# dusk-network/schnorr

Measured on NVIDIA B200. Metric: verifies_per_s, higher is better.
Workload: dtype u32

## Files before the change

### schnorr_b200/csrc/fq.cuh

```cuda
#pragma once
#include <cstdint>

#include "constants_gen.cuh"

#if defined(__CUDACC__)
#define SB_HD __host__ __device__ __forceinline__
#define SB_D __device__ __forceinline__
#else
#define SB_HD inline
#define SB_D inline
#endif

namespace sb200 {

#ifndef SB_Q1_SHORTCUT
#define SB_Q1_SHORTCUT 0
#endif

struct fq {
  uint32_t v[8];
};

#if !defined(__CUDA_ARCH__)
namespace emu {
// ... 60 lines not shown
      : "r"(a), "r"(b0), "r"(b2), "r"(b4), "r"(b6));
#else
  SB_COUNT(wide, 4);
  uint32_t c = emu::add_at(x, 8, 0, (uint64_t)a * b0, 0);
  c += emu::add_at(x, 8, 2, (uint64_t)a * b2, 0);
  c += emu::add_at(x, 8, 4, (uint64_t)a * b4, 0);
  c += emu::add_at(x, 8, 6, (uint64_t)a * b6, 0);
  ytop += c;
#endif
}

SB_HD void blk_mac_odd(uint32_t* y, uint32_t a, uint32_t b1, uint32_t b3, uint32_t b5, uint32_t b7) {
#if defined(__CUDA_ARCH__)
  asm("mad.lo.cc.u32 %0, %8, %9, %0;\n\t"
      "madc.hi.cc.u32 %1, %8, %9, %1;\n\t"
      "madc.lo.cc.u32 %2, %8, %10, %2;\n\t"
      "madc.hi.cc.u32 %3, %8, %10, %3;\n\t"
      "madc.lo.cc.u32 %4, %8, %11, %4;\n\t"
      "madc.hi.cc.u32 %5, %8, %11, %5;\n\t"
      "madc.lo.cc.u32 %6, %8, %12, %6;\n\t"
      "madc.hi.u32 %7, %8, %12, %7;"
      : "+r"(y[0]), "+r"(y[1]), "+r"(y[2]), "+r"(y[3]), "+r"(y[4]), "+r"(y[5]), "+r"(y[6]), "+r"(y[7])
      : "r"(a), "r"(b1), "r"(b3), "r"(b5), "r"(b7));
#else
  SB_COUNT(wide, 4);
  uint32_t c = emu::add_at(y, 8, 0, (uint64_t)a * b1, 0);
  c += emu::add_at(y, 8, 2, (uint64_t)a * b3, 0);
  c += emu::add_at(y, 8, 4, (uint64_t)a * b5, 0);
  c += emu::add_at(y, 8, 6, (uint64_t)a * b7, 0);
  (void)c;
#endif
}

SB_HD void blk_red_even_q(uint32_t* x, uint32_t& ytop, uint32_t m, uint32_t q2, uint32_t q4, uint32_t q6) {
#if defined(__CUDA_ARCH__)
  asm("mad.lo.cc.u32 %0, %7, %8, %0;\n\t"
      "madc.hi.cc.u32 %1, %7, %8, %1;\n\t"
      "madc.lo.cc.u32 %2, %7, %9, %2;\n\t"
      "madc.hi.cc.u32 %3, %7, %9, %3;\n\t"
      "madc.lo.cc.u32 %4, %7, %10, %4;\n\t"
      "madc.hi.cc.u32 %5, %7, %10, %5;\n\t"
      "addc.u32 %6, %6, 0;"
      : "+r"(x[2]), "+r"(x[3]), "+r"(x[4]), "+r"(x[5]), "+r"(x[6]), "+r"(x[7]), "+r"(ytop)
      : "r"(m), "r"(q2), "r"(q4), "r"(q6));
#else
  SB_COUNT(wide, 3);
  uint32_t c = emu::add_at(x, 8, 2, (uint64_t)m * q2, 0);
  c += emu::add_at(x, 8, 4, (uint64_t)m * q4, 0);
  c += emu::add_at(x, 8, 6, (uint64_t)m * q6, 0);
  ytop += c;
#endif
}

SB_HD void blk_red_odd_q(uint32_t* y, uint32_t m, uint32_t t0, uint32_t q3, uint32_t q5, uint32_t q7) {
#if defined(__CUDA_ARCH__)
  asm("{\n\t.reg .u32 h;\n\t"
      "min.u32 h, %8, 1;\n\t"
      "sub.u32 h, %8, h;\n\t"
      "add.cc.u32 %0, %0, %9;\n\t"
      "addc.cc.u32 %1, %1, h;\n\t"
      "madc.lo.cc.u32 %2, %8, %10, %2;\n\t"
      "madc.hi.cc.u32 %3, %8, %10, %3;\n\t"
      "madc.lo.cc.u32 %4, %8, %11, %4;\n\t"
      "madc.hi.cc.u32 %5, %8, %11, %5;\n\t"
      "madc.lo.cc.u32 %6, %8, %12, %6;\n\t"
      "madc.hi.u32 %7, %8, %12, %7;\n\t}"
      : "+r"(y[0]), "+r"(y[1]), "+r"(y[2]), "+r"(y[3]), "+r"(y[4]), "+r"(y[5]), "+r"(y[6]), "+r"(y[7])
      : "r"(m), "r"(t0), "r"(q3), "r"(q5), "r"(q7));
#else
  SB_COUNT(wide, 3);
  uint32_t hi1 = m - (m != 0 ? 1u : 0u);
  uint32_t c = emu::add_at(y, 8, 0, ((uint64_t)hi1 << 32) | t0, 0);
  c += emu::add_at(y, 8, 2, (uint64_t)m * q3, 0);
  c += emu::add_at(y, 8, 4, (uint64_t)m * q5, 0);
  c += emu::add_at(y, 8, 6, (uint64_t)m * q7, 0);
  (void)c;
#endif
}

SB_HD void blk_mac1c(uint32_t* acc, uint32_t a, uint32_t b0) {
#if defined(__CUDA_ARCH__)
  asm("mad.lo.cc.u32 %0, %3, %4, %0;\n\t"
      "madc.hi.cc.u32 %1, %3, %4, %1;\n\t"
      "addc.u32 %2, %2, 0;"
      : "+r"(acc[0]), "+r"(acc[1]), "+r"(acc[2])
      : "r"(a), "r"(b0));
#else
  SB_COUNT(wide, 1);
  acc[2] += emu::add_at(acc, 2, 0, (uint64_t)a * b0, 0);
#endif
}
SB_HD void blk_mac2c(uint32_t* acc, uint32_t a, uint32_t b0, uint32_t b1) {
#if defined(__CUDA_ARCH__)
  asm("mad.lo.cc.u32 %0, %5, %6, %0;\n\t"
      "madc.hi.cc.u32 %1, %5, %6, %1;\n\t"
      "madc.lo.cc.u32 %2, %5, %7, %2;\n\t"
      "madc.hi.cc.u32 %3, %5, %7, %3;\n\t"
      "addc.u32 %4, %4, 0;"
      : "+r"(acc[0]), "+r"(acc[1]), "+r"(acc[2]), "+r"(acc[3]), "+r"(acc[4])
      : "r"(a), "r"(b0), "r"(b1));
#else
  SB_COUNT(wide, 2);
  uint32_t c = emu::add_at(acc, 4, 0, (uint64_t)a * b0, 0);
  c += emu::add_at(acc, 4, 2, (uint64_t)a * b1, 0);
  acc[4] += c;
#endif
}
SB_HD void blk_mac3c(uint32_t* acc, uint32_t a, uint32_t b0, uint32_t b1, uint32_t b2) {
#if defined(__CUDA_ARCH__)
  asm("mad.lo.cc.u32 %0, %7, %8, %0;\n\t"
      "madc.hi.cc.u32 %1, %7, %8, %1;\n\t"
      "madc.lo.cc.u32 %2, %7, %9, %2;\n\t"
      "madc.hi.cc.u32 %3, %7, %9, %3;\n\t"
      "madc.lo.cc.u32 %4, %7, %10, %4;\n\t"
      "madc.hi.cc.u32 %5, %7, %10, %5;\n\t"
      "addc.u32 %6, %6, 0;"
      : "+r"(acc[0]), "+r"(acc[1]), "+r"(acc[2]), "+r"(acc[3]), "+r"(acc[4]), "+r"(acc[5]), "+r"(acc[6])
      : "r"(a), "r"(b0), "r"(b1), "r"(b2));
#else
  SB_COUNT(wide, 3);
  uint32_t c = emu::add_at(acc, 6, 0, (uint64_t)a * b0, 0);
  c += emu::add_at(acc, 6, 2, (uint64_t)a * b1, 0);
  c += emu::add_at(acc, 6, 4, (uint64_t)a * b2, 0);
  acc[6] += c;
#endif
}
SB_HD void blk_mac4c(uint32_t* acc, uint32_t a, uint32_t b0, uint32_t b1, uint32_t b2, uint32_t b3) {
  blk_mac_even(acc, acc[8], a, b0, b1, b2, b3);
}

SB_HD void blk_sqr_diag(uint32_t* t, const uint32_t* a) {
#if defined(__CUDA_ARCH__)
  asm("mad.lo.cc.u32 %0, %16, %16, %0;\n\t"
      "madc.hi.cc.u32 %1, %16, %16, %1;\n\t"
      "madc.lo.cc.u32 %2, %17, %17, %2;\n\t"
      "madc.hi.cc.u32 %3, %17, %17, %3;\n\t"
      "madc.lo.cc.u32 %4, %18, %18, %4;\n\t"
      "madc.hi.cc.u32 %5, %18, %18, %5;\n\t"
      "madc.lo.cc.u32 %6, %19, %19, %6;\n\t"
      "madc.hi.cc.u32 %7, %19, %19, %7;\n\t"
      "madc.lo.cc.u32 %8, %20, %20, %8;\n\t"
      "madc.hi.cc.u32 %9, %20, %20, %9;\n\t"
      "madc.lo.cc.u32 %10, %21, %21, %10;\n\t"
      "madc.hi.cc.u32 %11, %21, %21, %11;\n\t"
      "madc.lo.cc.u32 %12, %22, %22, %12;\n\t"
      "madc.hi.cc.u32 %13, %22, %22, %13;\n\t"
      "madc.lo.cc.u32 %14, %23, %23, %14;\n\t"
      "madc.hi.u32 %15, %23, %23, %15;"
      : "+r"(t[0]), "+r"(t[1]), "+r"(t[2]), "+r"(t[3]), "+r"(t[4]), "+r"(t[5]), "+r"(t[6]), "+r"(t[7]), "+r"(t[8]),
        "+r"(t[9]), "+r"(t[10]), "+r"(t[11]), "+r"(t[12]), "+r"(t[13]), "+r"(t[14]), "+r"(t[15])
      : "r"(a[0]), "r"(a[1]), "r"(a[2]), "r"(a[3]), "r"(a[4]), "r"(a[5]), "r"(a[6]), "r"(a[7]));
#else
  SB_COUNT(wide, 8);
  uint32_t c = 0;
  for (int i = 0; i < 8; i++) c += emu::add_at(t, 16, 2 * i, (uint64_t)a[i] * a[i], 0);
  (void)c;
#endif
}

SB_HD void merge_eo16(uint32_t* r, const uint32_t* e, const uint32_t* o) {
#if defined(__CUDA_ARCH__)
  r[0] = e[0];
  asm("add.cc.u32 %0, %15, %30;\n\t"
      "addc.cc.u32 %1, %16, %31;\n\t"
      "addc.cc.u32 %2, %17, %32;\n\t"
      "addc.cc.u32 %3, %18, %33;\n\t"
      "addc.cc.u32 %4, %19, %34;\n\t"
      "addc.cc.u32 %5, %20, %35;\n\t"
      "addc.cc.u32 %6, %21, %36;\n\t"
      "addc.cc.u32 %7, %22, %37;\n\t"
      "addc.cc.u32 %8, %23, %38;\n\t"
      "addc.cc.u32 %9, %24, %39;\n\t"
      "addc.cc.u32 %10, %25, %40;\n\t"
      "addc.cc.u32 %11, %26, %41;\n\t"
      "addc.cc.u32 %12, %27, %42;\n\t"
      "addc.cc.u32 %13, %28, %43;\n\t"
      "addc.u32 %14, %29, %44;"
      : "=r"(r[1]), "=r"(r[2]), "=r"(r[3]), "=r"(r[4]), "=r"(r[5]), "=r"(r[6]), "=r"(r[7]), "=r"(r[8]), "=r"(r[9]),
        "=r"(r[10]), "=r"(r[11]), "=r"(r[12]), "=r"(r[13]), "=r"(r[14]), "=r"(r[15])
      : "r"(e[1]), "r"(e[2]), "r"(e[3]), "r"(e[4]), "r"(e[5]), "r"(e[6]), "r"(e[7]), "r"(e[8]), "r"(e[9]), "r"(e[10]),
        "r"(e[11]), "r"(e[12]), "r"(e[13]), "r"(e[14]), "r"(e[15]), "r"(o[0]), "r"(o[1]), "r"(o[2]), "r"(o[3]), "r"(o[4]),
        "r"(o[5]), "r"(o[6]), "r"(o[7]), "r"(o[8]), "r"(o[9]), "r"(o[10]), "r"(o[11]), "r"(o[12]), "r"(o[13]), "r"(o[14]));
#else
  r[0] = e[0];
  uint64_t c = 0;
  for (int i = 1; i < 16; i++) {
    c += (uint64_t)e[i] + o[i - 1];
    r[i] = (uint32_t)c;
    c >>= 32;
  }
#endif
}

SB_HD uint32_t blk_fold_red_odd(uint32_t& x0, uint32_t xf, uint32_t tprev, uint32_t* y, uint32_t q1, uint32_t q3,
                                uint32_t q5, uint32_t q7) {
  uint32_t m;
#if defined(__CUDA_ARCH__)
  asm("{\n\t.reg .u32 t, h;\n\t"
      "add.cc.u32 t, %11, 0xffffffff;\n\t"
      "addc.cc.u32 %0, %0, %10;\n\t"
      "xor.b32 %9, %0, %12;\n\t"
      "add.u32 %9, %9, 1;\n\t"
      "min.u32 h, %9, 1;\n\t"
      "sub.u32 h, %9, h;\n\t"
      "addc.cc.u32 %1, %1, %0;\n\t"
      "addc.cc.u32 %2, %2, h;\n\t"
      "madc.lo.cc.u32 %3, %9, %13, %3;\n\t"
      "madc.hi.cc.u32 %4, %9, %13, %4;\n\t"
      "madc.lo.cc.u32 %5, %9, %14, %5;\n\t"
      "madc.hi.cc.u32 %6, %9, %14, %6;\n\t"
      "madc.lo.cc.u32 %7, %9, %15, %7;\n\t"
      "madc.hi.u32 %8, %9, %15, %8;\n\t}"
      : "+r"(x0), "+r"(y[0]), "+r"(y[1]), "+r"(y[2]), "+r"(y[3]), "+r"(y[4]), "+r"(y[5]), "+r"(y[6]), "+r"(y[7]), "=&r"(m)
      : "r"(xf), "r"(tprev), "r"(q1), "r"(q3), "r"(q5), "r"(q7));
#else
  SB_COUNT(wide, 4);
  uint64_t t = (uint64_t)x0 + xf + (tprev != 0 ? 1u : 0u);
  x0 = (uint32_t)t;
  uint32_t c = (uint32_t)(t >> 32);
  m = 0u - x0;
  SB_COUNT(wide, -1);
  (void)q1;
  c = emu::add_at(y, 8, 0, ((uint64_t)(m - (m != 0 ? 1u : 0u)) << 32) | x0, c);
  c += emu::add_at(y, 8, 2, (uint64_t)m * q3, 0);
  c += emu::add_at(y, 8, 4, (uint64_t)m * q5, 0);
  c += emu::add_at(y, 8, 6, (uint64_t)m * q7, 0);
  (void)c;
#endif
  return m;
}

SB_HD uint32_t add8(uint32_t* r, const uint32_t* a, const uint32_t* b) {
  uint32_t c;
#if defined(__CUDA_ARCH__)
  asm("add.cc.u32 %0, %9, %17;\n\t"
      "addc.cc.u32 %1, %10, %18;\n\t"
      "addc.cc.u32 %2, %11, %19;\n\t"
      "addc.cc.u32 %3, %12, %20;\n\t"
      "addc.cc.u32 %4, %13, %21;\n\t"
      "addc.cc.u32 %5, %14, %22;\n\t"
      "addc.cc.u32 %6, %15, %23;\n\t"
      "addc.cc.u32 %7, %16, %24;\n\t"
      "addc.u32 %8, 0, 0;"
      : "=r"(r[0]), "=r"(r[1]), "=r"(r[2]), "=r"(r[3]), "=r"(r[4]), "=r"(r[5]), "=r"(r[6]), "=r"(r[7]), "=r"(c)
      : "r"(a[0]), "r"(a[1]), "r"(a[2]), "r"(a[3]), "r"(a[4]), "r"(a[5]), "r"(a[6]), "r"(a[7]), "r"(b[0]), "r"(b[1]),
        "r"(b[2]), "r"(b[3]), "r"(b[4]), "r"(b[5]), "r"(b[6]), "r"(b[7]));
#else
  uint64_t t = 0;
  for (int i = 0; i < 8; i++) {
    t += (uint64_t)a[i] + b[i];
    r[i] = (uint32_t)t;
    t >>= 32;
  }
  c = (uint32_t)t;
#endif
  return c;
}

SB_HD void add8c(uint32_t* r, const uint32_t* a, const uint32_t* b, uint32_t t) {
#if defined(__CUDA_ARCH__)
  asm("{\n\t.reg .u32 t;\n\t"
      "add.cc.u32 t, %24, 0xffffffff;\n\t"
      "addc.cc.u32 %0, %8, %16;\n\t"
      "addc.cc.u32 %1, %9, %17;\n\t"
      "addc.cc.u32 %2, %10, %18;\n\t"
      "addc.cc.u32 %3, %11, %19;\n\t"
      "addc.cc.u32 %4, %12, %20;\n\t"
      "addc.cc.u32 %5, %13, %21;\n\t"
      "addc.cc.u32 %6, %14, %22;\n\t"
      "addc.u32 %7, %15, %23;\n\t}"
      : "=r"(r[0]), "=r"(r[1]), "=r"(r[2]), "=r"(r[3]), "=r"(r[4]), "=r"(r[5]), "=r"(r[6]), "=r"(r[7])
      : "r"(a[0]), "r"(a[1]), "r"(a[2]), "r"(a[3]), "r"(a[4]), "r"(a[5]), "r"(a[6]), "r"(a[7]), "r"(b[0]), "r"(b[1]),
        "r"(b[2]), "r"(b[3]), "r"(b[4]), "r"(b[5]), "r"(b[6]), "r"(b[7]), "r"(t));
#else
  uint64_t c = t != 0 ? 1 : 0;
  for (int i = 0; i < 8; i++) {
    c += (uint64_t)a[i] + b[i];
    r[i] = (uint32_t)c;
    c >>= 32;
  }
// ... 164 lines not shown
  return mont_reduce16(T);
#endif
  uint32_t X[8], Y[8], xf = 0, tprev = 0;
#pragma unroll
  for (int i = 0; i < 8; i++) X[i] = Y[i] = 0;
  const uint32_t q1 = SB_FQ_MOD(1), q2 = SB_FQ_MOD(2), q3 = SB_FQ_MOD(3), q4 = SB_FQ_MOD(4), q5 = SB_FQ_MOD(5),
                 q6 = SB_FQ_MOD(6), q7 = SB_FQ_MOD(7);
#pragma unroll
  for (int i = 0; i < 8; i++) {
    uint32_t ai = a.v[i];
    blk_fold_mac_odd(X[0], xf, tprev, Y, ai, b.v[1], b.v[3], b.v[5], b.v[7]);
    blk_mac_even(X, Y[7], ai, b.v[0], b.v[2], b.v[4], b.v[6]);
    tprev = X[0];
#if defined(__CUDA_ARCH__) && SB_FQ_MOD_IMM
    uint32_t m;
    asm("xor.b32 %0, %1, %2;\n\tadd.u32 %0, %0, 1;" : "=r"(m) : "r"(tprev), "r"(q1));
#else
    uint32_t m = (tprev ^ q1) + 1u;
#endif
    blk_red_even_q(X, Y[7], m, q2, q4, q6);
#if SB_Q1_SHORTCUT
    blk_red_odd_q(Y, m, tprev, q3, q5, q7);
#else
    blk_mac_odd(Y, m, q1, q3, q5, q7);
#endif
    xf = X[1];
    uint32_t nx[8], ny[8];
#pragma unroll
    for (int k = 0; k < 8; k++) nx[k] = Y[k];
#pragma unroll
    for (int k = 0; k < 6; k++) ny[k] = X[k + 2];
    ny[6] = 0;
    ny[7] = 0;
#pragma unroll
    for (int k = 0; k < 8; k++) {
      X[k] = nx[k];
      Y[k] = ny[k];
    }
  }
  fq r;
  uint32_t s[8] = {xf, Y[0], Y[1], Y[2], Y[3], Y[4], Y[5], Y[6]};
  add8c(r.v, X, s, tprev);
  cond_sub_p<FqP>(r.v);
  return r;
}

SB_HD fq mont_reduce16(const uint32_t* t) {
  uint32_t X[8], Y[8], xf = 0, tprev = 0;
#pragma unroll
  for (int i = 0; i < 8; i++) {
    X[i] = t[i];
    Y[i] = 0;
  }
  const uint32_t q1 = SB_FQ_MOD(1), q2 = SB_FQ_MOD(2), q3 = SB_FQ_MOD(3), q4 = SB_FQ_MOD(4), q5 = SB_FQ_MOD(5),
                 q6 = SB_FQ_MOD(6), q7 = SB_FQ_MOD(7);
#pragma unroll
  for (int i = 0; i < 8; i++) {
    uint32_t m = blk_fold_red_odd(X[0], xf, tprev, Y, q1, q3, q5, q7);
    tprev = X[0];
    blk_red_even_q(X, Y[7], m, q2, q4, q6);
    xf = X[1];
    uint32_t nx[8], ny[8];
#pragma unroll
    for (int k = 0; k < 8; k++) nx[k] = Y[k];
#pragma unroll
    for (int k = 0; k < 6; k++) ny[k] = X[k + 2];
    ny[6] = 0;
    ny[7] = 0;
#pragma unroll
    for (int k = 0; k < 8; k++) {
      X[k] = nx[k];
      Y[k] = ny[k];
    }
  }
  fq v, r;
  uint32_t s[8] = {xf, Y[0], Y[1], Y[2], Y[3], Y[4], Y[5], Y[6]};
  add8c(v.v, X, s, tprev);
  add8(r.v, v.v, t + 8);
  cond_sub_p<FqP>(r.v);
  return r;
}

SB_HD fq fq_sqr_inl(const fq& x) {
  SB_COUNT(fq_sqr, 1);
  const uint32_t* a = x.v;
  uint32_t E[16], O[16];
#pragma unroll
  for (int i = 0; i < 16; i++) E[i] = O[i] = 0;
  blk_mac4c(O + 0, a[0], a[1], a[3], a[5], a[7]);
  blk_mac3c(E + 2, a[0], a[2], a[4], a[6]);
  blk_mac3c(O + 2, a[1], a[2], a[4], a[6]);
  blk_mac3c(E + 4, a[1], a[3], a[5], a[7]);
  blk_mac3c(O + 4, a[2], a[3], a[5], a[7]);
  blk_mac2c(E + 6, a[2], a[4], a[6]);
  blk_mac2c(O + 6, a[3], a[4], a[6]);
  blk_mac2c(E + 8, a[3], a[5], a[7]);
  blk_mac2c(O + 8, a[4], a[5], a[7]);
  blk_mac1c(E + 10, a[4], a[6]);
  blk_mac1c(O + 10, a[5], a[6]);
  blk_mac1c(E + 12, a[5], a[7]);
  blk_mac1c(O + 12, a[6], a[7]);
  uint32_t S[16], T[16];
  merge_eo16(S, E, O);
  T[0] = S[0] << 1;
#pragma unroll
  for (int i = 1; i < 16; i++) T[i] = (S[i] << 1) | (S[i - 1] >> 31);
  blk_sqr_diag(T, a);
  return mont_reduce16(T);
}

SB_HD void mul_wide16(uint32_t* T, const uint32_t* a, const uint32_t* b) {
  uint32_t E[18], O[18];
#pragma unroll
  for (int i = 0; i < 18; i++) E[i] = O[i] = 0;
#pragma unroll
  for (int i = 0; i < 8; i++) {
    if ((i & 1) == 0) {
      blk_mac4c(E + i, a[i], b[0], b[2], b[4], b[6]);
      blk_mac4c(O + i, a[i], b[1], b[3], b[5], b[7]);
    } else {
      blk_mac4c(O + i - 1, a[i], b[0], b[2], b[4], b[6]);
      blk_mac4c(E + i + 1, a[i], b[1], b[3], b[5], b[7]);
    }
  }
  merge_eo16(T, E, O);
}

SB_HD void acc17(uint32_t* S, const uint32_t* T) {
#if defined(__CUDA_ARCH__)
  asm("add.cc.u32 %0, %0, %17;\n\t"
      "addc.cc.u32 %1, %1, %18;\n\t"
      "addc.cc.u32 %2, %2, %19;\n\t"
      "addc.cc.u32 %3, %3, %20;\n\t"
      "addc.cc.u32 %4, %4, %21;\n\t"
      "addc.cc.u32 %5, %5, %22;\n\t"
      "addc.cc.u32 %6, %6, %23;\n\t"
      "addc.cc.u32 %7, %7, %24;\n\t"
      "addc.cc.u32 %8, %8, %25;\n\t"
      "addc.cc.u32 %9, %9, %26;\n\t"
      "addc.cc.u32 %10, %10, %27;\n\t"
      "addc.cc.u32 %11, %11, %28;\n\t"
      "addc.cc.u32 %12, %12, %29;\n\t"
      "addc.cc.u32 %13, %13, %30;\n\t"
      "addc.cc.u32 %14, %14, %31;\n\t"
      "addc.cc.u32 %15, %15, %32;\n\t"
      "addc.u32 %16, %16, 0;"
      : "+r"(S[0]), "+r"(S[1]), "+r"(S[2]), "+r"(S[3]), "+r"(S[4]), "+r"(S[5]), "+r"(S[6]), "+r"(S[7]), "+r"(S[8]),
        "+r"(S[9]), "+r"(S[10]), "+r"(S[11]), "+r"(S[12]), "+r"(S[13]), "+r"(S[14]), "+r"(S[15]), "+r"(S[16])
      : "r"(T[0]), "r"(T[1]), "r"(T[2]), "r"(T[3]), "r"(T[4]), "r"(T[5]), "r"(T[6]), "r"(T[7]), "r"(T[8]), "r"(T[9]),
        "r"(T[10]), "r"(T[11]), "r"(T[12]), "r"(T[13]), "r"(T[14]), "r"(T[15]));
#else
  uint64_t c = 0;
  for (int i = 0; i < 16; i++) {
    c += (uint64_t)S[i] + T[i];
    S[i] = (uint32_t)c;
    c >>= 32;
  }
  S[16] += (uint32_t)c;
#endif
}

SB_HD fq mont_reduce17(const uint32_t* S) {
  uint32_t X[8], Y[8], xf = 0, tprev = 0;
#pragma unroll
  for (int i = 0; i < 8; i++) {
    X[i] = S[i];
    Y[i] = 0;
  }
  const uint32_t q1 = SB_FQ_MOD(1), q2 = SB_FQ_MOD(2), q3 = SB_FQ_MOD(3), q4 = SB_FQ_MOD(4), q5 = SB_FQ_MOD(5),
                 q6 = SB_FQ_MOD(6), q7 = SB_FQ_MOD(7);
#pragma unroll
  for (int i = 0; i < 8; i++) {
    uint32_t m = blk_fold_red_odd(X[0], xf, tprev, Y, q1, q3, q5, q7);
    tprev = X[0];
    blk_red_even_q(X, Y[7], m, q2, q4, q6);
    xf = X[1];
    uint32_t nx[8], ny[8];
#pragma unroll
    for (int k = 0; k < 8; k++) nx[k] = Y[k];
#pragma unroll
    for (int k = 0; k < 6; k++) ny[k] = X[k + 2];
    ny[6] = 0;
    ny[7] = 0;
#pragma unroll
    for (int k = 0; k < 8; k++) {
      X[k] = nx[k];
      Y[k] = ny[k];
    }
  }
  fq v, r;
  uint32_t s[8] = {xf, Y[0], Y[1], Y[2], Y[3], Y[4], Y[5], Y[6]};
  add8c(v.v, X, s, tprev);
  uint32_t top = S[16] + add8(r.v, v.v, S + 8);
  uint32_t t[8], q2x[8];
#pragma unroll
  for (int i = 0; i < 8; i++) q2x[i] = (FqP::p(i) << 1) | (i ? FqP::p(i - 1) >> 31 : 0u);
  uint32_t borrow = sub8(t, r.v, q2x);
  bool ge = (top != 0) | (borrow == 0);
#pragma unroll
  for (int i = 0; i < 8; i++) r.v[i] = ge ? t[i] : r.v[i];
  cond_sub_p<FqP>(r.v);
  return r;
}

SB_HD void merge_eo17(uint32_t* S, const uint32_t* E, const uint32_t* O) {
  S[0] = E[0];
#if defined(__CUDA_ARCH__)
  asm("add.cc.u32 %0, %16, %32;\n\t"
      "addc.cc.u32 %1, %17, %33;\n\t"
      "addc.cc.u32 %2, %18, %34;\n\t"
      "addc.cc.u32 %3, %19, %35;\n\t"
      "addc.cc.u32 %4, %20, %36;\n\t"
      "addc.cc.u32 %5, %21, %37;\n\t"
      "addc.cc.u32 %6, %22, %38;\n\t"
      "addc.cc.u32 %7, %23, %39;\n\t"
      "addc.cc.u32 %8, %24, %40;\n\t"
      "addc.cc.u32 %9, %25, %41;\n\t"
      "addc.cc.u32 %10, %26, %42;\n\t"
      "addc.cc.u32 %11, %27, %43;\n\t"
      "addc.cc.u32 %12, %28, %44;\n\t"
      "addc.cc.u32 %13, %29, %45;\n\t"
      "addc.cc.u32 %14, %30, %46;\n\t"
      "addc.u32 %15, %31, %47;"
      : "=r"(S[1]), "=r"(S[2]), "=r"(S[3]), "=r"(S[4]), "=r"(S[5]), "=r"(S[6]), "=r"(S[7]), "=r"(S[8]), "=r"(S[9]), "=r"(S[10]),
        "=r"(S[11]), "=r"(S[12]), "=r"(S[13]), "=r"(S[14]), "=r"(S[15]), "=r"(S[16])
      : "r"(E[1]), "r"(E[2]), "r"(E[3]), "r"(E[4]), "r"(E[5]), "r"(E[6]), "r"(E[7]), "r"(E[8]), "r"(E[9]), "r"(E[10]), "r"(E[11]),
// ... 223 lines not shown
```

Measured before the change: 28.79 million.

## Interleave field squaring with Montgomery reduction using pre-doubled operands

Replaces the separate 16-word product, doubling and diagonal pass in fq_sqr_inl with a row-by-row interleaved square-and-reduce (CIOS style). Pre-doubled limbs of a fold the cross-term doubling into the multiplicands, and the reduction helpers now return their top carry so it can be fed into the next row. This removes the merge and shift passes and the wide 16-limb intermediate, lowering register pressure and instruction count. In exchange the carry handling is more intricate, and the product terms are no longer triangular-only, so some of the squaring savings on multiplies are given up.

```diff
diff --git a/schnorr_b200/csrc/fq.cuh b/schnorr_b200/csrc/fq.cuh
--- a/schnorr_b200/csrc/fq.cuh
+++ b/schnorr_b200/csrc/fq.cuh
@@ -136,20 +136,22 @@
 #endif
 }
 
-SB_HD void blk_red_odd_q(uint32_t* y, uint32_t m, uint32_t t0, uint32_t q3, uint32_t q5, uint32_t q7) {
+SB_HD uint32_t blk_red_odd_q(uint32_t* y, uint32_t m, uint32_t t0, uint32_t q3, uint32_t q5, uint32_t q7) {
+  uint32_t ovf;
 #if defined(__CUDA_ARCH__)
   asm("{\n\t.reg .u32 h;\n\t"
-      "min.u32 h, %8, 1;\n\t"
-      "sub.u32 h, %8, h;\n\t"
-      "add.cc.u32 %0, %0, %9;\n\t"
+      "min.u32 h, %9, 1;\n\t"
+      "sub.u32 h, %9, h;\n\t"
+      "add.cc.u32 %0, %0, %10;\n\t"
       "addc.cc.u32 %1, %1, h;\n\t"
-      "madc.lo.cc.u32 %2, %8, %10, %2;\n\t"
-      "madc.hi.cc.u32 %3, %8, %10, %3;\n\t"
-      "madc.lo.cc.u32 %4, %8, %11, %4;\n\t"
-      "madc.hi.cc.u32 %5, %8, %11, %5;\n\t"
-      "madc.lo.cc.u32 %6, %8, %12, %6;\n\t"
-      "madc.hi.u32 %7, %8, %12, %7;\n\t}"
-      : "+r"(y[0]), "+r"(y[1]), "+r"(y[2]), "+r"(y[3]), "+r"(y[4]), "+r"(y[5]), "+r"(y[6]), "+r"(y[7])
+      "madc.lo.cc.u32 %2, %9, %11, %2;\n\t"
+      "madc.hi.cc.u32 %3, %9, %11, %3;\n\t"
+      "madc.lo.cc.u32 %4, %9, %12, %4;\n\t"
+      "madc.hi.cc.u32 %5, %9, %12, %5;\n\t"
+      "madc.lo.cc.u32 %6, %9, %13, %6;\n\t"
+      "madc.hi.cc.u32 %7, %9, %13, %7;\n\t"
+      "addc.u32 %8, 0, 0;\n\t}"
+      : "+r"(y[0]), "+r"(y[1]), "+r"(y[2]), "+r"(y[3]), "+r"(y[4]), "+r"(y[5]), "+r"(y[6]), "+r"(y[7]), "=r"(ovf)
       : "r"(m), "r"(t0), "r"(q3), "r"(q5), "r"(q7));
 #else
   SB_COUNT(wide, 3);
@@ -158,39 +160,40 @@
   c += emu::add_at(y, 8, 2, (uint64_t)m * q3, 0);
   c += emu::add_at(y, 8, 4, (uint64_t)m * q5, 0);
   c += emu::add_at(y, 8, 6, (uint64_t)m * q7, 0);
-  (void)c;
-#endif
-}
-
-SB_HD void blk_mac1c(uint32_t* acc, uint32_t a, uint32_t b0) {
+  ovf = c;
+#endif
+  return ovf;
+}
+
+SB_HD void blk_mac1c(uint32_t* acc, uint32_t& top, uint32_t a, uint32_t b0) {
 #if defined(__CUDA_ARCH__)
   asm("mad.lo.cc.u32 %0, %3, %4, %0;\n\t"
       "madc.hi.cc.u32 %1, %3, %4, %1;\n\t"
       "addc.u32 %2, %2, 0;"
-      : "+r"(acc[0]), "+r"(acc[1]), "+r"(acc[2])
+      : "+r"(acc[0]), "+r"(acc[1]), "+r"(top)
       : "r"(a), "r"(b0));
 #else
   SB_COUNT(wide, 1);
-  acc[2] += emu::add_at(acc, 2, 0, (uint64_t)a * b0, 0);
-#endif
-}
-SB_HD void blk_mac2c(uint32_t* acc, uint32_t a, uint32_t b0, uint32_t b1) {
+  top += emu::add_at(acc, 2, 0, (uint64_t)a * b0, 0);
+#endif
+}
+SB_HD void blk_mac2c(uint32_t* acc, uint32_t& top, uint32_t a, uint32_t b0, uint32_t b1) {
 #if defined(__CUDA_ARCH__)
   asm("mad.lo.cc.u32 %0, %5, %6, %0;\n\t"
       "madc.hi.cc.u32 %1, %5, %6, %1;\n\t"
       "madc.lo.cc.u32 %2, %5, %7, %2;\n\t"
       "madc.hi.cc.u32 %3, %5, %7, %3;\n\t"
       "addc.u32 %4, %4, 0;"
-      : "+r"(acc[0]), "+r"(acc[1]), "+r"(acc[2]), "+r"(acc[3]), "+r"(acc[4])
+      : "+r"(acc[0]), "+r"(acc[1]), "+r"(acc[2]), "+r"(acc[3]), "+r"(top)
       : "r"(a), "r"(b0), "r"(b1));
 #else
   SB_COUNT(wide, 2);
   uint32_t c = emu::add_at(acc, 4, 0, (uint64_t)a * b0, 0);
   c += emu::add_at(acc, 4, 2, (uint64_t)a * b1, 0);
-  acc[4] += c;
-#endif
-}
-SB_HD void blk_mac3c(uint32_t* acc, uint32_t a, uint32_t b0, uint32_t b1, uint32_t b2) {
+  top += c;
+#endif
+}
+SB_HD void blk_mac3c(uint32_t* acc, uint32_t& top, uint32_t a, uint32_t b0, uint32_t b1, uint32_t b2) {
 #if defined(__CUDA_ARCH__)
   asm("mad.lo.cc.u32 %0, %7, %8, %0;\n\t"
       "madc.hi.cc.u32 %1, %7, %8, %1;\n\t"
@@ -199,45 +202,61 @@
       "madc.lo.cc.u32 %4, %7, %10, %4;\n\t"
       "madc.hi.cc.u32 %5, %7, %10, %5;\n\t"
       "addc.u32 %6, %6, 0;"
-      : "+r"(acc[0]), "+r"(acc[1]), "+r"(acc[2]), "+r"(acc[3]), "+r"(acc[4]), "+r"(acc[5]), "+r"(acc[6])
+      : "+r"(acc[0]), "+r"(acc[1]), "+r"(acc[2]), "+r"(acc[3]), "+r"(acc[4]), "+r"(acc[5]), "+r"(top)
       : "r"(a), "r"(b0), "r"(b1), "r"(b2));
 #else
   SB_COUNT(wide, 3);
   uint32_t c = emu::add_at(acc, 6, 0, (uint64_t)a * b0, 0);
   c += emu::add_at(acc, 6, 2, (uint64_t)a * b1, 0);
   c += emu::add_at(acc, 6, 4, (uint64_t)a * b2, 0);
-  acc[6] += c;
+  top += c;
 #endif
 }
 SB_HD void blk_mac4c(uint32_t* acc, uint32_t a, uint32_t b0, uint32_t b1, uint32_t b2, uint32_t b3) {
   blk_mac_even(acc, acc[8], a, b0, b1, b2, b3);
 }
 
-SB_HD void blk_sqr_diag(uint32_t* t, const uint32_t* a) {
-#if defined(__CUDA_ARCH__)
-  asm("mad.lo.cc.u32 %0, %16, %16, %0;\n\t"
-      "madc.hi.cc.u32 %1, %16, %16, %1;\n\t"
-      "madc.lo.cc.u32 %2, %17, %17, %2;\n\t"
-      "madc.hi.cc.u32 %3, %17, %17, %3;\n\t"
-      "madc.lo.cc.u32 %4, %18, %18, %4;\n\t"
-      "madc.hi.cc.u32 %5, %18, %18, %5;\n\t"
-      "madc.lo.cc.u32 %6, %19, %19, %6;\n\t"
-      "madc.hi.cc.u32 %7, %19, %19, %7;\n\t"
-      "madc.lo.cc.u32 %8, %20, %20, %8;\n\t"
-      "madc.hi.cc.u32 %9, %20, %20, %9;\n\t"
-      "madc.lo.cc.u32 %10, %21, %21, %10;\n\t"
-      "madc.hi.cc.u32 %11, %21, %21, %11;\n\t"
-      "madc.lo.cc.u32 %12, %22, %22, %12;\n\t"
-      "madc.hi.cc.u32 %13, %22, %22, %13;\n\t"
-      "madc.lo.cc.u32 %14, %23, %23, %14;\n\t"
-      "madc.hi.u32 %15, %23, %23, %15;"
-      : "+r"(t[0]), "+r"(t[1]), "+r"(t[2]), "+r"(t[3]), "+r"(t[4]), "+r"(t[5]), "+r"(t[6]), "+r"(t[7]), "+r"(t[8]),
-        "+r"(t[9]), "+r"(t[10]), "+r"(t[11]), "+r"(t[12]), "+r"(t[13]), "+r"(t[14]), "+r"(t[15])
-      : "r"(a[0]), "r"(a[1]), "r"(a[2]), "r"(a[3]), "r"(a[4]), "r"(a[5]), "r"(a[6]), "r"(a[7]));
-#else
-  SB_COUNT(wide, 8);
-  uint32_t c = 0;
-  for (int i = 0; i < 8; i++) c += emu::add_at(t, 16, 2 * i, (uint64_t)a[i] * a[i], 0);
+SB_HD void blk_mac1(uint32_t* acc, uint32_t a, uint32_t b0) {
+#if defined(__CUDA_ARCH__)
+  asm("mad.lo.cc.u32 %0, %2, %3, %0;\n\t"
+      "madc.hi.u32 %1, %2, %3, %1;"
+      : "+r"(acc[0]), "+r"(acc[1])
+      : "r"(a), "r"(b0));
+#else
+  SB_COUNT(wide, 1);
+  (void)emu::add_at(acc, 2, 0, (uint64_t)a * b0, 0);
+#endif
+}
+SB_HD void blk_mac2(uint32_t* acc, uint32_t a, uint32_t b0, uint32_t b1) {
+#if defined(__CUDA_ARCH__)
+  asm("mad.lo.cc.u32 %0, %4, %5, %0;\n\t"
+      "madc.hi.cc.u32 %1, %4, %5, %1;\n\t"
+      "madc.lo.cc.u32 %2, %4, %6, %2;\n\t"
+      "madc.hi.u32 %3, %4, %6, %3;"
+      : "+r"(acc[0]), "+r"(acc[1]), "+r"(acc[2]), "+r"(acc[3])
+      : "r"(a), "r"(b0), "r"(b1));
+#else
+  SB_COUNT(wide, 2);
+  uint32_t c = emu::add_at(acc, 4, 0, (uint64_t)a * b0, 0);
+  c += emu::add_at(acc, 4, 2, (uint64_t)a * b1, 0);
+  (void)c;
+#endif
+}
+SB_HD void blk_mac3(uint32_t* acc, uint32_t a, uint32_t b0, uint32_t b1, uint32_t b2) {
+#if defined(__CUDA_ARCH__)
+  asm("mad.lo.cc.u32 %0, %6, %7, %0;\n\t"
+      "madc.hi.cc.u32 %1, %6, %7, %1;\n\t"
+      "madc.lo.cc.u32 %2, %6, %8, %2;\n\t"
+      "madc.hi.cc.u32 %3, %6, %8, %3;\n\t"
+      "madc.lo.cc.u32 %4, %6, %9, %4;\n\t"
+      "madc.hi.u32 %5, %6, %9, %5;"
+      : "+r"(acc[0]), "+r"(acc[1]), "+r"(acc[2]), "+r"(acc[3]), "+r"(acc[4]), "+r"(acc[5])
+      : "r"(a), "r"(b0), "r"(b1), "r"(b2));
+#else
+  SB_COUNT(wide, 3);
+  uint32_t c = emu::add_at(acc, 6, 0, (uint64_t)a * b0, 0);
+  c += emu::add_at(acc, 6, 2, (uint64_t)a * b1, 0);
+  c += emu::add_at(acc, 6, 4, (uint64_t)a * b2, 0);
   (void)c;
 #endif
 }
@@ -277,25 +296,27 @@
 }
 
 SB_HD uint32_t blk_fold_red_odd(uint32_t& x0, uint32_t xf, uint32_t tprev, uint32_t* y, uint32_t q1, uint32_t q3,
-                                uint32_t q5, uint32_t q7) {
+                                uint32_t q5, uint32_t q7, uint32_t& ovf) {
   uint32_t m;
 #if defined(__CUDA_ARCH__)
   asm("{\n\t.reg .u32 t, h;\n\t"
-      "add.cc.u32 t, %11, 0xffffffff;\n\t"
-      "addc.cc.u32 %0, %0, %10;\n\t"
-      "xor.b32 %9, %0, %12;\n\t"
+      "add.cc.u32 t, %12, 0xffffffff;\n\t"
+      "addc.cc.u32 %0, %0, %11;\n\t"
+      "xor.b32 %9, %0, %13;\n\t"
       "add.u32 %9, %9, 1;\n\t"
       "min.u32 h, %9, 1;\n\t"
       "sub.u32 h, %9, h;\n\t"
       "addc.cc.u32 %1, %1, %0;\n\t"
       "addc.cc.u32 %2, %2, h;\n\t"
-      "madc.lo.cc.u32 %3, %9, %13, %3;\n\t"
-      "madc.hi.cc.u32 %4, %9, %13, %4;\n\t"
-      "madc.lo.cc.u32 %5, %9, %14, %5;\n\t"
-      "madc.hi.cc.u32 %6, %9, %14, %6;\n\t"
-      "madc.lo.cc.u32 %7, %9, %15, %7;\n\t"
-      "madc.hi.u32 %8, %9, %15, %8;\n\t}"
-      : "+r"(x0), "+r"(y[0]), "+r"(y[1]), "+r"(y[2]), "+r"(y[3]), "+r"(y[4]), "+r"(y[5]), "+r"(y[6]), "+r"(y[7]), "=&r"(m)
+      "madc.lo.cc.u32 %3, %9, %14, %3;\n\t"
+      "madc.hi.cc.u32 %4, %9, %14, %4;\n\t"
+      "madc.lo.cc.u32 %5, %9, %15, %5;\n\t"
+      "madc.hi.cc.u32 %6, %9, %15, %6;\n\t"
+      "madc.lo.cc.u32 %7, %9, %16, %7;\n\t"
+      "madc.hi.cc.u32 %8, %9, %16, %8;\n\t"
+      "addc.u32 %10, 0, 0;\n\t}"
+      : "+r"(x0), "+r"(y[0]), "+r"(y[1]), "+r"(y[2]), "+r"(y[3]), "+r"(y[4]), "+r"(y[5]), "+r"(y[6]), "+r"(y[7]), "=&r"(m),
+        "=r"(ovf)
       : "r"(xf), "r"(tprev), "r"(q1), "r"(q3), "r"(q5), "r"(q7));
 #else
   SB_COUNT(wide, 4);
@@ -309,7 +330,7 @@
   c += emu::add_at(y, 8, 2, (uint64_t)m * q3, 0);
   c += emu::add_at(y, 8, 4, (uint64_t)m * q5, 0);
   c += emu::add_at(y, 8, 6, (uint64_t)m * q7, 0);
-  (void)c;
+  ovf = c;
 #endif
   return m;
 }
@@ -584,7 +605,8 @@
                  q6 = SB_FQ_MOD(6), q7 = SB_FQ_MOD(7);
 #pragma unroll
   for (int i = 0; i < 8; i++) {
-    uint32_t m = blk_fold_red_odd(X[0], xf, tprev, Y, q1, q3, q5, q7);
+    uint32_t ovf;
+    uint32_t m = blk_fold_red_odd(X[0], xf, tprev, Y, q1, q3, q5, q7, ovf);
     tprev = X[0];
     blk_red_even_q(X, Y[7], m, q2, q4, q6);
     xf = X[1];
@@ -612,29 +634,69 @@
 SB_HD fq fq_sqr_inl(const fq& x) {
   SB_COUNT(fq_sqr, 1);
   const uint32_t* a = x.v;
-  uint32_t E[16], O[16];
-#pragma unroll
-  for (int i = 0; i < 16; i++) E[i] = O[i] = 0;
-  blk_mac4c(O + 0, a[0], a[1], a[3], a[5], a[7]);
-  blk_mac3c(E + 2, a[0], a[2], a[4], a[6]);
-  blk_mac3c(O + 2, a[1], a[2], a[4], a[6]);
-  blk_mac3c(E + 4, a[1], a[3], a[5], a[7]);
-  blk_mac3c(O + 4, a[2], a[3], a[5], a[7]);
-  blk_mac2c(E + 6, a[2], a[4], a[6]);
-  blk_mac2c(O + 6, a[3], a[4], a[6]);
-  blk_mac2c(E + 8, a[3], a[5], a[7]);
-  blk_mac2c(O + 8, a[4], a[5], a[7]);
-  blk_mac1c(E + 10, a[4], a[6]);
-  blk_mac1c(O + 10, a[5], a[6]);
-  blk_mac1c(E + 12, a[5], a[7]);
-  blk_mac1c(O + 12, a[6], a[7]);
-  uint32_t S[16], T[16];
-  merge_eo16(S, E, O);
-  T[0] = S[0] << 1;
-#pragma unroll
-  for (int i = 1; i < 16; i++) T[i] = (S[i] << 1) | (S[i - 1] >> 31);
-  blk_sqr_diag(T, a);
-  return mont_reduce16(T);
+  uint32_t s1[8], d[8];
+#pragma unroll
+  for (int j = 1; j < 8; j++) {
+    s1[j] = a[j] << 1;
+    d[j] = s1[j] | (a[j - 1] >> 31);
+  }
+  uint32_t X[8], Y[8], xf = 0, tprev = 0;
+#pragma unroll
+  for (int i = 0; i < 8; i++) X[i] = Y[i] = 0;
+  const uint32_t q1 = SB_FQ_MOD(1), q2 = SB_FQ_MOD(2), q3 = SB_FQ_MOD(3), q4 = SB_FQ_MOD(4), q5 = SB_FQ_MOD(5),
+                 q6 = SB_FQ_MOD(6), q7 = SB_FQ_MOD(7);
+#pragma unroll
+  for (int i = 0; i < 8; i++) {
+    const uint32_t ai = a[i];
+    uint32_t b[8];
+#pragma unroll
+    for (int j = 0; j < 8; j++) b[j] = j < i ? 0u : j == i ? ai : j == i + 1 ? s1[j] : d[j];
+    uint32_t z = 0, ovf, m;
+    switch ((i + 1) >> 1) {
+      case 0: blk_mac_even(X, z, ai, b[0], b[2], b[4], b[6]); break;
+      case 1: blk_mac3c(X + 2, z, ai, b[2], b[4], b[6]); break;
+      case 2: blk_mac2c(X + 4, z, ai, b[4], b[6]); break;
+      case 3: blk_mac1c(X + 6, z, ai, b[6]); break;
+      default: break;
+    }
+    switch (i >> 1) {
+      case 0: blk_mac_odd(Y, ai, b[1], b[3], b[5], b[7]); break;
+      case 1: blk_mac3(Y + 2, ai, b[3], b[5], b[7]); break;
+      case 2: blk_mac2(Y + 4, ai, b[5], b[7]); break;
+      default: blk_mac1(Y + 6, ai, b[7]); break;
+    }
+    if (i == 0) {
+      tprev = X[0];
+#if defined(__CUDA_ARCH__) && SB_FQ_MOD_IMM
+      asm("xor.b32 %0, %1, %2;\n\tadd.u32 %0, %0, 1;" : "=r"(m) : "r"(tprev), "r"(q1));
+#else
+      m = (tprev ^ q1) + 1u;
+#endif
+      ovf = blk_red_odd_q(Y, m, tprev, q3, q5, q7);
+    } else {
+      m = blk_fold_red_odd(X[0], xf, tprev, Y, q1, q3, q5, q7, ovf);
+      tprev = X[0];
+    }
+    blk_red_even_q(X, z, m, q2, q4, q6);
+    xf = X[1];
+    uint32_t nx[8], ny[8];
+#pragma unroll
+    for (int k = 0; k < 8; k++) nx[k] = Y[k];
+#pragma unroll
+    for (int k = 0; k < 6; k++) ny[k] = X[k + 2];
+    ny[6] = z;
+    ny[7] = ovf;
+#pragma unroll
+    for (int k = 0; k < 8; k++) {
+      X[k] = nx[k];
+      Y[k] = ny[k];
+    }
+  }
+  fq r;
+  uint32_t s[8] = {xf, Y[0], Y[1], Y[2], Y[3], Y[4], Y[5], Y[6]};
+  add8c(r.v, X, s, tprev);
+  cond_sub_p<FqP>(r.v);
+  return r;
 }
 
 SB_HD void mul_wide16(uint32_t* T, const uint32_t* a, const uint32_t* b) {
@@ -699,7 +761,8 @@
                  q6 = SB_FQ_MOD(6), q7 = SB_FQ_MOD(7);
 #pragma unroll
   for (int i = 0; i < 8; i++) {
-    uint32_t m = blk_fold_red_odd(X[0], xf, tprev, Y, q1, q3, q5, q7);
+    uint32_t ovf;
+    uint32_t m = blk_fold_red_odd(X[0], xf, tprev, Y, q1, q3, q5, q7, ovf);
     tprev = X[0];
     blk_red_even_q(X, Y[7], m, q2, q4, q6);
     xf = X[1];
```

After: 29.32 million, median of 6. 1.02x the previous value.

## Interleave Montgomery reduction into field squaring and simplify m computation

Applied to the files above, without the earlier changes.

Rewrites fq_sqr to fold the Montgomery reduction row by row into the squaring product, using a pre-doubled operand so cross terms and diagonals are accumulated together instead of building a 16-limb product, doubling it and reducing it separately. This removes the wide intermediate, the shift pass and the separate diagonal pass, and should lower register pressure. It also replaces the xor/add computation of m with a negation, which drops the q1 operand and assumes a modulus-specific identity. The new schedule is intricate, and the per-row carry bounds must hold for correctness.

```diff
diff --git a/schnorr_b200/csrc/fq.cuh b/schnorr_b200/csrc/fq.cuh
--- a/schnorr_b200/csrc/fq.cuh
+++ b/schnorr_b200/csrc/fq.cuh
@@ -162,35 +162,35 @@
 #endif
 }
 
-SB_HD void blk_mac1c(uint32_t* acc, uint32_t a, uint32_t b0) {
+SB_HD void blk_mac1(uint32_t* acc, uint32_t& top, uint32_t a, uint32_t b0) {
 #if defined(__CUDA_ARCH__)
   asm("mad.lo.cc.u32 %0, %3, %4, %0;\n\t"
       "madc.hi.cc.u32 %1, %3, %4, %1;\n\t"
       "addc.u32 %2, %2, 0;"
-      : "+r"(acc[0]), "+r"(acc[1]), "+r"(acc[2])
+      : "+r"(acc[0]), "+r"(acc[1]), "+r"(top)
       : "r"(a), "r"(b0));
 #else
   SB_COUNT(wide, 1);
-  acc[2] += emu::add_at(acc, 2, 0, (uint64_t)a * b0, 0);
-#endif
-}
-SB_HD void blk_mac2c(uint32_t* acc, uint32_t a, uint32_t b0, uint32_t b1) {
+  top += emu::add_at(acc, 2, 0, (uint64_t)a * b0, 0);
+#endif
+}
+SB_HD void blk_mac2(uint32_t* acc, uint32_t& top, uint32_t a, uint32_t b0, uint32_t b1) {
 #if defined(__CUDA_ARCH__)
   asm("mad.lo.cc.u32 %0, %5, %6, %0;\n\t"
       "madc.hi.cc.u32 %1, %5, %6, %1;\n\t"
       "madc.lo.cc.u32 %2, %5, %7, %2;\n\t"
       "madc.hi.cc.u32 %3, %5, %7, %3;\n\t"
       "addc.u32 %4, %4, 0;"
-      : "+r"(acc[0]), "+r"(acc[1]), "+r"(acc[2]), "+r"(acc[3]), "+r"(acc[4])
+      : "+r"(acc[0]), "+r"(acc[1]), "+r"(acc[2]), "+r"(acc[3]), "+r"(top)
       : "r"(a), "r"(b0), "r"(b1));
 #else
   SB_COUNT(wide, 2);
   uint32_t c = emu::add_at(acc, 4, 0, (uint64_t)a * b0, 0);
   c += emu::add_at(acc, 4, 2, (uint64_t)a * b1, 0);
-  acc[4] += c;
-#endif
-}
-SB_HD void blk_mac3c(uint32_t* acc, uint32_t a, uint32_t b0, uint32_t b1, uint32_t b2) {
+  top += c;
+#endif
+}
+SB_HD void blk_mac3(uint32_t* acc, uint32_t& top, uint32_t a, uint32_t b0, uint32_t b1, uint32_t b2) {
 #if defined(__CUDA_ARCH__)
   asm("mad.lo.cc.u32 %0, %7, %8, %0;\n\t"
       "madc.hi.cc.u32 %1, %7, %8, %1;\n\t"
@@ -199,47 +199,24 @@
       "madc.lo.cc.u32 %4, %7, %10, %4;\n\t"
       "madc.hi.cc.u32 %5, %7, %10, %5;\n\t"
       "addc.u32 %6, %6, 0;"
-      : "+r"(acc[0]), "+r"(acc[1]), "+r"(acc[2]), "+r"(acc[3]), "+r"(acc[4]), "+r"(acc[5]), "+r"(acc[6])
+      : "+r"(acc[0]), "+r"(acc[1]), "+r"(acc[2]), "+r"(acc[3]), "+r"(acc[4]), "+r"(acc[5]), "+r"(top)
       : "r"(a), "r"(b0), "r"(b1), "r"(b2));
 #else
   SB_COUNT(wide, 3);
   uint32_t c = emu::add_at(acc, 6, 0, (uint64_t)a * b0, 0);
   c += emu::add_at(acc, 6, 2, (uint64_t)a * b1, 0);
   c += emu::add_at(acc, 6, 4, (uint64_t)a * b2, 0);
-  acc[6] += c;
+  top += c;
 #endif
 }
 SB_HD void blk_mac4c(uint32_t* acc, uint32_t a, uint32_t b0, uint32_t b1, uint32_t b2, uint32_t b3) {
   blk_mac_even(acc, acc[8], a, b0, b1, b2, b3);
 }
-
-SB_HD void blk_sqr_diag(uint32_t* t, const uint32_t* a) {
-#if defined(__CUDA_ARCH__)
-  asm("mad.lo.cc.u32 %0, %16, %16, %0;\n\t"
-      "madc.hi.cc.u32 %1, %16, %16, %1;\n\t"
-      "madc.lo.cc.u32 %2, %17, %17, %2;\n\t"
-      "madc.hi.cc.u32 %3, %17, %17, %3;\n\t"
-      "madc.lo.cc.u32 %4, %18, %18, %4;\n\t"
-      "madc.hi.cc.u32 %5, %18, %18, %5;\n\t"
-      "madc.lo.cc.u32 %6, %19, %19, %6;\n\t"
-      "madc.hi.cc.u32 %7, %19, %19, %7;\n\t"
-      "madc.lo.cc.u32 %8, %20, %20, %8;\n\t"
-      "madc.hi.cc.u32 %9, %20, %20, %9;\n\t"
-      "madc.lo.cc.u32 %10, %21, %21, %10;\n\t"
-      "madc.hi.cc.u32 %11, %21, %21, %11;\n\t"
-      "madc.lo.cc.u32 %12, %22, %22, %12;\n\t"
-      "madc.hi.cc.u32 %13, %22, %22, %13;\n\t"
-      "madc.lo.cc.u32 %14, %23, %23, %14;\n\t"
-      "madc.hi.u32 %15, %23, %23, %15;"
-      : "+r"(t[0]), "+r"(t[1]), "+r"(t[2]), "+r"(t[3]), "+r"(t[4]), "+r"(t[5]), "+r"(t[6]), "+r"(t[7]), "+r"(t[8]),
-        "+r"(t[9]), "+r"(t[10]), "+r"(t[11]), "+r"(t[12]), "+r"(t[13]), "+r"(t[14]), "+r"(t[15])
-      : "r"(a[0]), "r"(a[1]), "r"(a[2]), "r"(a[3]), "r"(a[4]), "r"(a[5]), "r"(a[6]), "r"(a[7]));
-#else
-  SB_COUNT(wide, 8);
-  uint32_t c = 0;
-  for (int i = 0; i < 8; i++) c += emu::add_at(t, 16, 2 * i, (uint64_t)a[i] * a[i], 0);
-  (void)c;
-#endif
+SB_HD void blk_mac_n(uint32_t* acc, uint32_t& top, uint32_t a, const uint32_t* b, int n) {
+  if (n == 4) blk_mac_even(acc, top, a, b[0], b[1], b[2], b[3]);
+  if (n == 3) blk_mac3(acc, top, a, b[0], b[1], b[2]);
+  if (n == 2) blk_mac2(acc, top, a, b[0], b[1]);
+  if (n == 1) blk_mac1(acc, top, a, b[0]);
 }
 
 SB_HD void merge_eo16(uint32_t* r, const uint32_t* e, const uint32_t* o) {
@@ -276,27 +253,25 @@
 #endif
 }
 
-SB_HD uint32_t blk_fold_red_odd(uint32_t& x0, uint32_t xf, uint32_t tprev, uint32_t* y, uint32_t q1, uint32_t q3,
-                                uint32_t q5, uint32_t q7) {
+SB_HD uint32_t blk_fold_red_odd(uint32_t& x0, uint32_t xf, uint32_t tprev, uint32_t* y, uint32_t q3, uint32_t q5, uint32_t q7) {
   uint32_t m;
 #if defined(__CUDA_ARCH__)
   asm("{\n\t.reg .u32 t, h;\n\t"
       "add.cc.u32 t, %11, 0xffffffff;\n\t"
       "addc.cc.u32 %0, %0, %10;\n\t"
-      "xor.b32 %9, %0, %12;\n\t"
-      "add.u32 %9, %9, 1;\n\t"
+      "sub.u32 %9, 0, %0;\n\t"
       "min.u32 h, %9, 1;\n\t"
       "sub.u32 h, %9, h;\n\t"
       "addc.cc.u32 %1, %1, %0;\n\t"
       "addc.cc.u32 %2, %2, h;\n\t"
-      "madc.lo.cc.u32 %3, %9, %13, %3;\n\t"
-      "madc.hi.cc.u32 %4, %9, %13, %4;\n\t"
-      "madc.lo.cc.u32 %5, %9, %14, %5;\n\t"
-      "madc.hi.cc.u32 %6, %9, %14, %6;\n\t"
-      "madc.lo.cc.u32 %7, %9, %15, %7;\n\t"
-      "madc.hi.u32 %8, %9, %15, %8;\n\t}"
+      "madc.lo.cc.u32 %3, %9, %12, %3;\n\t"
+      "madc.hi.cc.u32 %4, %9, %12, %4;\n\t"
+      "madc.lo.cc.u32 %5, %9, %13, %5;\n\t"
+      "madc.hi.cc.u32 %6, %9, %13, %6;\n\t"
+      "madc.lo.cc.u32 %7, %9, %14, %7;\n\t"
+      "madc.hi.u32 %8, %9, %14, %8;\n\t}"
       : "+r"(x0), "+r"(y[0]), "+r"(y[1]), "+r"(y[2]), "+r"(y[3]), "+r"(y[4]), "+r"(y[5]), "+r"(y[6]), "+r"(y[7]), "=&r"(m)
-      : "r"(xf), "r"(tprev), "r"(q1), "r"(q3), "r"(q5), "r"(q7));
+      : "r"(xf), "r"(tprev), "r"(q3), "r"(q5), "r"(q7));
 #else
   SB_COUNT(wide, 4);
   uint64_t t = (uint64_t)x0 + xf + (tprev != 0 ? 1u : 0u);
@@ -304,7 +279,6 @@
   uint32_t c = (uint32_t)(t >> 32);
   m = 0u - x0;
   SB_COUNT(wide, -1);
-  (void)q1;
   c = emu::add_at(y, 8, 0, ((uint64_t)(m - (m != 0 ? 1u : 0u)) << 32) | x0, c);
   c += emu::add_at(y, 8, 2, (uint64_t)m * q3, 0);
   c += emu::add_at(y, 8, 4, (uint64_t)m * q5, 0);
@@ -580,11 +554,11 @@
     X[i] = t[i];
     Y[i] = 0;
   }
-  const uint32_t q1 = SB_FQ_MOD(1), q2 = SB_FQ_MOD(2), q3 = SB_FQ_MOD(3), q4 = SB_FQ_MOD(4), q5 = SB_FQ_MOD(5),
+  const uint32_t q2 = SB_FQ_MOD(2), q3 = SB_FQ_MOD(3), q4 = SB_FQ_MOD(4), q5 = SB_FQ_MOD(5),
                  q6 = SB_FQ_MOD(6), q7 = SB_FQ_MOD(7);
 #pragma unroll
   for (int i = 0; i < 8; i++) {
-    uint32_t m = blk_fold_red_odd(X[0], xf, tprev, Y, q1, q3, q5, q7);
+    uint32_t m = blk_fold_red_odd(X[0], xf, tprev, Y, q3, q5, q7);
     tprev = X[0];
     blk_red_even_q(X, Y[7], m, q2, q4, q6);
     xf = X[1];
@@ -612,29 +586,77 @@
 SB_HD fq fq_sqr_inl(const fq& x) {
   SB_COUNT(fq_sqr, 1);
   const uint32_t* a = x.v;
-  uint32_t E[16], O[16];
-#pragma unroll
-  for (int i = 0; i < 16; i++) E[i] = O[i] = 0;
-  blk_mac4c(O + 0, a[0], a[1], a[3], a[5], a[7]);
-  blk_mac3c(E + 2, a[0], a[2], a[4], a[6]);
-  blk_mac3c(O + 2, a[1], a[2], a[4], a[6]);
-  blk_mac3c(E + 4, a[1], a[3], a[5], a[7]);
-  blk_mac3c(O + 4, a[2], a[3], a[5], a[7]);
-  blk_mac2c(E + 6, a[2], a[4], a[6]);
-  blk_mac2c(O + 6, a[3], a[4], a[6]);
-  blk_mac2c(E + 8, a[3], a[5], a[7]);
-  blk_mac2c(O + 8, a[4], a[5], a[7]);
-  blk_mac1c(E + 10, a[4], a[6]);
-  blk_mac1c(O + 10, a[5], a[6]);
-  blk_mac1c(E + 12, a[5], a[7]);
-  blk_mac1c(O + 12, a[6], a[7]);
-  uint32_t S[16], T[16];
-  merge_eo16(S, E, O);
-  T[0] = S[0] << 1;
-#pragma unroll
-  for (int i = 1; i < 16; i++) T[i] = (S[i] << 1) | (S[i - 1] >> 31);
-  blk_sqr_diag(T, a);
-  return mont_reduce16(T);
+  uint32_t e[8], d[8];
+#pragma unroll
+  for (int k = 1; k < 8; k++) e[k] = a[k] << 1;
+#pragma unroll
+  for (int k = 2; k < 8; k++) d[k] = e[k] | (a[k - 1] >> 31);
+  const uint32_t q2 = SB_FQ_MOD(2), q3 = SB_FQ_MOD(3), q4 = SB_FQ_MOD(4), q5 = SB_FQ_MOD(5),
+                 q6 = SB_FQ_MOD(6), q7 = SB_FQ_MOD(7);
+  uint32_t X[8], Y[8], xf, tprev;
+  {
+    SB_COUNT(wide, 7);
+    const uint64_t p00 = (uint64_t)a[0] * a[0];
+    tprev = (uint32_t)p00;
+    xf = (uint32_t)(p00 >> 32);
+    uint32_t m;
+#if defined(__CUDA_ARCH__) && SB_FQ_MOD_IMM
+    asm("sub.u32 %0, 0, %1;" : "=r"(m) : "r"(tprev));
+#else
+    m = 0u - tprev;
+#endif
+    X[0] = tprev;
+    X[1] = m - (m != 0 ? 1u : 0u);
+    const uint32_t qo[3] = {q3, q5, q7}, qe[3] = {q2, q4, q6};
+#pragma unroll
+    for (int j = 0; j < 3; j++) {
+      const uint64_t po = (uint64_t)m * qo[j], pe = (uint64_t)m * qe[j];
+      X[2 * j + 2] = (uint32_t)po;
+      X[2 * j + 3] = (uint32_t)(po >> 32);
+      Y[2 * j] = (uint32_t)pe;
+      Y[2 * j + 1] = (uint32_t)(pe >> 32);
+    }
+    Y[6] = Y[7] = 0;
+  }
+#pragma unroll
+  for (int i = 0; i < 8; i++) {
+    if (i > 0) {
+      const uint32_t m = blk_fold_red_odd(X[0], xf, tprev, Y, q3, q5, q7);
+      tprev = X[0];
+      blk_red_even_q(X, Y[7], m, q2, q4, q6);
+      xf = X[1];
+      uint32_t nx[8], ny[8];
+#pragma unroll
+      for (int k = 0; k < 8; k++) nx[k] = Y[k];
+#pragma unroll
+      for (int k = 0; k < 6; k++) ny[k] = X[k + 2];
+      ny[6] = 0;
+      ny[7] = 0;
+#pragma unroll
+      for (int k = 0; k < 8; k++) {
+        X[k] = nx[k];
+        Y[k] = ny[k];
+      }
+    }
+    uint32_t b[8];
+#pragma unroll
+    for (int k = i; k < 8; k++) b[k] = k == i ? a[i] : k == i + 1 ? e[k] : d[k];
+    const int k_odd = i | 1, k_even = i < 2 ? 2 : (i + 1) & ~1;
+    uint32_t bo[4], be[3];
+#pragma unroll
+    for (int k = k_odd; k < 8; k += 2) bo[(k - k_odd) / 2] = b[k];
+    blk_mac_n(X + k_odd - 1, Y[7], a[i], bo, (9 - k_odd) / 2);
+    if (k_even < 8) {
+#pragma unroll
+      for (int k = k_even; k < 8; k += 2) be[(k - k_even) / 2] = b[k];
+      blk_mac_n(Y + k_even - 2, Y[6], a[i], be, (8 - k_even) / 2);
+    }
+  }
+  fq r;
+  uint32_t s[8] = {xf, Y[0], Y[1], Y[2], Y[3], Y[4], Y[5], Y[6]};
+  add8c(r.v, X, s, tprev);
+  cond_sub_p<FqP>(r.v);
+  return r;
 }
 
 SB_HD void mul_wide16(uint32_t* T, const uint32_t* a, const uint32_t* b) {
@@ -695,11 +717,11 @@
     X[i] = S[i];
     Y[i] = 0;
   }
-  const uint32_t q1 = SB_FQ_MOD(1), q2 = SB_FQ_MOD(2), q3 = SB_FQ_MOD(3), q4 = SB_FQ_MOD(4), q5 = SB_FQ_MOD(5),
+  const uint32_t q2 = SB_FQ_MOD(2), q3 = SB_FQ_MOD(3), q4 = SB_FQ_MOD(4), q5 = SB_FQ_MOD(5),
                  q6 = SB_FQ_MOD(6), q7 = SB_FQ_MOD(7);
 #pragma unroll
   for (int i = 0; i < 8; i++) {
-    uint32_t m = blk_fold_red_odd(X[0], xf, tprev, Y, q1, q3, q5, q7);
+    uint32_t m = blk_fold_red_odd(X[0], xf, tprev, Y, q3, q5, q7);
     tprev = X[0];
     blk_red_even_q(X, Y[7], m, q2, q4, q6);
     xf = X[1];
```

New measurement: 28.83 million before, 29.39 million after (median of 6 runs). 1.9% higher.
